# phaistos-networks/Trinity

Hardware: AMD Instinct MI355X
Metric: queries/sec (higher is better)
Workload: dtype u32

## Files before the change

### trinity_amd/csrc/k_score.hpp

```cpp
#pragma once
#include "k_match.hpp"

#ifndef TRI_SCORE_TILE
#define TRI_SCORE_TILE 4096
#endif
constexpr uint32_t SCORE_TILE = TRI_SCORE_TILE;
constexpr uint32_t TOPK_CAP = TOPK_MAX + AND_WG;

struct TopK {
        double s[TOPK_CAP];
        uint32_t d[TOPK_CAP];
        uint32_t n;
        uint32_t full;
        double thr_s;
        uint32_t thr_d;
};

__device__ __forceinline__ bool better(const double s1, const uint32_t d1, const double s2, const uint32_t d2) {
        return s1 > s2 || (s1 == s2 && d1 < d2);
}

__device__ void topk_prune(TopK &tk, const uint32_t k, uint32_t *scan) {
        const uint32_t tid = threadIdx.x;
        const uint32_t n = uni(tk.n);
// ... 337 lines not shown
                                                       float *__restrict__ top_scores, uint32_t *__restrict__ top_counts) {
        __shared__ TopK tk;
        __shared__ uint32_t scan[8];
        const uint32_t tid = threadIdx.x;
        for (uint32_t slot = blockIdx.x; slot < nq; slot += gridDim.x) {
                const DevQuery q = plan[slot];
                if (q.qid == 0xffffffffu)
                        continue;
                tk.n = 0;
                tk.full = 0;
                __syncthreads();
                for (uint32_t t = 0; t < q.ntasks; ++t) {
                        const uint32_t tix = q.first_task + t;
                        const uint32_t c = part_counts[tix];
                        for (uint32_t base = 0; base < c; base += AND_WG) {
                                const uint32_t i = base + tid;
                                const bool v = i < c;
                                topk_offer(tk, k, v, v ? part_scores[(uint64_t)tix * k + i] : 0.0, v ? part_docs[(uint64_t)tix * k + i] : 0u, scan);
                        }
                }
                topk_prune(tk, k, scan);
                const uint32_t n = uni(tk.n);
                for (uint32_t i = tid; i < k; i += AND_WG) {
                        top_docs[(uint64_t)q.qid * k + i] = i < n ? tk.d[i] : 0u;
                        top_scores[(uint64_t)q.qid * k + i] = i < n ? (float)tk.s[i] : 0.0f;
                }
                if (uni(tid >> 6) == 0)
                        top_counts[q.qid] = n;
                __syncthreads();
        }
}

__global__ void k_query_counts(const DevQuery *__restrict__ plan, const uint32_t *__restrict__ counts_by_task, const uint32_t nq,
                               uint64_t *__restrict__ qcounts) {
        const uint32_t s = blockIdx.x * blockDim.x + threadIdx.x;
        if (s >= nq)
                return;
        const DevQuery q = plan[s];
        if (q.qid == 0xffffffffu)
                return;
        uint64_t c = 0;
        for (uint32_t t = 0; t < q.ntasks; ++t)
                c += counts_by_task[q.first_task + t];
        qcounts[q.qid] = c;
}

struct DevSource {
        const DevQuery *plan;
        const uint32_t *slot_of_query;
        const uint32_t *part_docs;
        const double *part_scores;
        const uint32_t *part_counts;
        const uint64_t *qcounts;
};
__global__ __launch_bounds__(AND_WG) void k_topk_merge_sources(const DevSource *__restrict__ src, const uint32_t nsrc, const uint32_t nq, const uint32_t k,
                                                               uint32_t *__restrict__ top_docs, float *__restrict__ top_scores,
                                                               uint32_t *__restrict__ top_counts, uint64_t *__restrict__ counts) {
        __shared__ TopK tk;
        __shared__ uint32_t scan[8];
        const uint32_t tid = threadIdx.x;
        for (uint32_t qi = blockIdx.x; qi < nq; qi += gridDim.x) {
                tk.n = 0;
                tk.full = 0;
                __syncthreads();
                uint64_t total = 0;
                for (uint32_t s = 0; s < nsrc; ++s) {
                        const DevSource S = src[s];
// ... 134 lines not shown
```

### trinity_amd/csrc/trinity_hip.hip

```cpp
#include "../../include/trinity_hip.h"
#include <chrono>
#include <hip/hip_runtime.h>

#include <algorithm>
#include <array>
#include <cmath>
#include <cstdarg>
#include <cstdio>
#include <cstring>
#include <ctime>
#include <unistd.h>
#include <dlfcn.h>
#include <memory>
#include <mutex>
#include <numeric>
#include <string>
#include <thread>
#include <unordered_map>
#include <functional>
#include <vector>

static thread_local char g_err[512] = "";
static int fail(int code, const char *fmt, ...) {
        va_list ap;
// ... 256 lines not shown
struct tri_filter {
        DevRef dev;
        tri_index *ix = nullptr;
        Pooled<uint32_t> d_bits;
        size_t words = 0;
        ~tri_filter() {
                if (dev)
                        hipSetDevice(dev->device);
        }
};
struct tri_column {
        DevRef dev;
        tri_index *ix = nullptr;
        DevMem<uint32_t> d_values;
        uint32_t n = 0;
        ~tri_column() {
                if (dev)
                        hipSetDevice(dev->device);
        }
};
static size_t filter_words(const tri_index *ix) { return ((size_t)ix->max_doc / SPAN_BITS + 2) * SPAN_WORDS; }

enum BatchEvent { EV_UP, EV_START, EV_PLANE_ROWS, EV_DENSE, EV_PSET, EV_PROBE, EV_CAND, EV_FUSED, EV_PLANES, EV_PHRASE, EV_TREE, EV_END, EV_COUNT };

struct tri_batch : BatchPlan {
        DevRef dev;
        tri_index *ix = nullptr;
        uint32_t flags, topk;
        int similarity = TRI_SIM_BM25;
        size_t nq;
        Pinned<uint8_t> pinned;
        Pooled<uint8_t> d_arena;
        PooledEvent ev[EV_COUNT];
        Pooled<uint32_t> d_sparse;
        Pooled<uint32_t> d_out;
        Pooled<uint32_t> d_rich_allow;
        DevMem<uint64_t> d_hashes;
        Pooled<uint32_t> d_part_docs;
        Pooled<double> d_part_scores, d_all_scores;
        Pooled<uint32_t> d_rich_present;
        Pooled<uint16_t> d_rich_freq;
        Pooled<uint16_t> d_rich_freq_wide;
        Pooled<uint32_t> d_rich_present_hi, d_rich_allow_hi;
        DevMem<uint16_t> d_rich_pool;
        DevMem<uint8_t> d_rich_plen;
        DevMem<uint64_t> d_rich_payload;
        Pooled<double> d_pscore;
        Pooled<uint32_t> d_tree_scratch;
        Pooled<double> d_tree_scores;
        Pooled<uint32_t> d_scat_docs;
        Pooled<uint8_t> d_filter_tab;
        Pooled<uint32_t> d_filter_rows;
        Pooled<uint8_t> d_rank_block;
        Pooled<uint32_t> d_facet_rows;
        PooledEvent facet_ev[2];
        Pooled<uint64_t> d_order_block;
        DevMem<DevOrderGroup> d_order_groups;
        PooledEvent order_ev[2];
        template <class T>
        T *dev_at(const Span<T> &s) const {
                return reinterpret_cast<T *>(d_arena + s.off);
        }
        template <class T>
        T *dev_opt(const Span<T> &s) const {
                return s.empty() ? nullptr : dev_at(s);
        }
// ... 704 lines not shown
                        plan_lock = std::unique_lock<std::mutex>(dev->planners[0].mu);
                }
                tri_dev::PlanCtx &pc = dev->planners[which];
                if (nq >= 1024 && !pc.pool) {
                        const unsigned budget = host_cpu_budget();
                        const unsigned fair = budget >= 10 ? std::min(16u, (budget - 4) / tri_dev::PLAN_CTXS) : budget >= 4 ? 2u : 1u;
                        const unsigned want = dev->opt.plan_threads ? (unsigned)std::min<uint64_t>(dev->opt.plan_threads, 64) : fair;
                        if (want > 1) {
                                try {
                                        DevLock g(dev->mu);
                                        pc.pool = std::make_unique<HostPool>(want, dev->opt.plan_pin != 0, (unsigned)dev->opt.plan_hot_us, which, tri_dev::PLAN_CTXS, dev->plan_anchor, dev->opt.plan_pin == 2);
                                        if (dev->plan_anchor < 0)
                                                dev->plan_anchor = pc.pool->anchor();
                                } catch (...) {
                                }
                        }
                }
                rc = plan_batch(*ix, env, in, pc.pool.get(), [&](size_t bytes) { return b->pinned.alloc(dev, bytes); }, *b, err, &pc.frag_cache);
        } catch (const std::bad_alloc &) {
                return fail(TRI_ERR_NOMEM, "tri_batch_create: out of host memory");
        }
        if (rc != TRI_OK)
                return fail(rc, "%s", err.c_str());
        if (!b->last_unsupported.empty())
                fail(TRI_ERR_UNSUPPORTED, "%s", b->last_unsupported.c_str());
        return TRI_OK;
}

static size_t batch_arena(tri_batch *b, uint8_t *base, size_t *zero_from) {
        const size_t nt = b->tasks.size(), np = b->plan.size(), nq = b->nq, topk = b->topk;
        const bool scored = batch_scored(b), rich = batch_rich(b), scatter = b->pscatter_queries;
        Carver carve{base, b->block_bytes};
        carve(b->d_counts, (nt + 1) * 4);
        carve(b->d_ticket, TICKET_BYTES);
        carve(b->d_build, (b->plane_terms.size() + 1) * 8);
        carve(b->d_qthr, (np + 1) * 8, b->n_planes + b->n_planes8 != 0);
        carve(b->d_part_counts, (nt + 1) * 4, scored);
        carve(b->d_score_order, (nt + 1) * 4, scored);
        carve(b->d_task_hits, (nt + 1) * 4, rich);
        carve(b->d_task_pos_base, (nt + 1) * 8, rich);
        carve(b->d_scat_off, (nt + 1) * 4, scatter);
        carve(b->d_scat_cnt, (nt + 1) * 4, scatter);
        carve(b->d_scat_list, (b->pscatter_queries + 1) * 4, scatter);
        *zero_from = carve.at;
        carve(b->d_qcounts, (nq + 1) * 8);
        carve(b->d_top_counts, (nq + 1) * 4, scored);
        carve(b->d_top_docs, (nq * topk + 1) * 4, scored);
        carve(b->d_top_scores, (nq * topk + 1) * 4, scored);
        return carve.at;
}

static int create_arena(tri_batch *b) {
        tri_dev *dev = b->dev;
        size_t a_zero = 0;
        const size_t a = batch_arena(b, nullptr, &a_zero);
        HIP_TRY(b->d_arena.alloc(dev, a + 256));
        batch_arena(b, b->d_arena, &a_zero);
        if (b->pscatter_queries) {
                if (b->pscatter_docs + 64 > 0xffffffffull)
                        return fail(TRI_ERR_UNSUPPORTED, "tri_batch_create: the unions' terms without a plane hold more than 2^32 documents");
                b->scat_cap = (uint32_t)b->pscatter_docs;
                HIP_TRY(b->d_scat_docs.alloc(dev, ((size_t)b->scat_cap + 64) * 4));
        }
        for (PooledEvent &e : b->ev)
                HIP_TRY(e.take(dev));
        if (b->block_bytes)
                HIP_TRY(hipMemcpyAsync(b->d_arena, b->block, b->block_bytes, hipMemcpyHostToDevice, dev->stream_up));
        HIP_TRY(hipMemsetAsync(b->d_arena + a_zero, 0, a - a_zero, dev->stream_up));
        return TRI_OK;
}

static size_t tree_scratch(tri_batch *b, uint32_t *base) {
        const size_t plw = b->plw, nterms = b->tree_terms.size(), nhid = b->tree_hidden.size(), nchunks = (plw + TREE_CHUNK_WORDS - 1) / TREE_CHUNK_WORDS;
        Carver carve{reinterpret_cast<uint8_t *>(base), 0, 4};
        carve(b->d_tree_rows, nterms * PL_PLANES * plw * 4);
        carve(b->d_tree_prows, nhid * plw * 4);
        carve(b->d_tree_qbits, (size_t)b->n_tree * plw * 4);
// ... 95 lines not shown
        };
        auto b = std::make_unique<tri_batch>();
        b->ix = ix;
        b->dev.retain(dev);
        b->flags = flags;
        b->topk = topk;
        b->similarity = similarity;
        b->nq = nq;
        const PlanInput in{prog, prog_len, queries, nq, weights, flags, topk, similarity};
        if (const int rc = create_plan(b.get(), in))
                return rc;
        dbg_lap(0);
        DevLock dev_lock(dev->mu);
        if (const int rc = create_arena(b.get()))
                return rc;
        dbg_lap(1);
        if (const int rc = create_buffers(b.get(), in, dbg_lap))
                return rc;
        HIP_TRY(hipEventRecord(b->ev[EV_UP], dev->stream_up));
        create_info(b.get());
        b->info.create_ms = (float)std::chrono::duration<double, std::milli>(std::chrono::steady_clock::now() - t_create).count();
        if (dbg_create)
                fprintf(stderr, "[tri create] nq %zu: plan %.3f  arena+copy %.3f  planes/sparse %.3f  out(%.1f MB) %.3f  rest %.3f  total %.3f ms\n", nq, dbg_t[0], dbg_t[1] - dbg_t[0],
                        dbg_t[2] - dbg_t[1], (double)b->out_capacity * 4 / 1e6, dbg_t[3] - dbg_t[2], b->info.create_ms - dbg_t[3], b->info.create_ms);
        *out = b.release();
        return TRI_OK;
}

extern "C" void tri_batch_destroy(tri_batch *b) {
        delete b;
}


static FilterSel filter_sel(const tri_batch *b) {
        if (b->filter_rows.empty())
                return FilterSel{nullptr, nullptr, nullptr, 0u};
        return FilterSel{b->d_filter_rows, (const uint32_t *)b->d_filter_tab.get(), b->dev_at(b->tasks), (uint32_t)filter_words(b->ix)};
}
template <class F>
struct FilteredKernel;
template <class... A>
struct FilteredKernel<void (*)(A...)> {
        using type = void (*)(A..., FilterSel);
};
template <class Pick, class... Args>
static void tri_launch_matching(const tri_batch *b, const int kernel, const int variant, Pick pick, const dim3 grid, const dim3 block, const hipStream_t stream, Args &&...args) {
        const FilterSel fsel = filter_sel(b);
        if (!fsel.rows)
                return tri_launch(b->ix->codec, pick, grid, block, stream, std::forward<Args>(args)...);
        using Plain = decltype(+pick(std::integral_constant<int, CODEC_GOOGLE>()));
        const auto twin = reinterpret_cast<typename FilteredKernel<Plain>::type>(const_cast<void *>(filtered_kernel(kernel, b->ix->codec == TRI_CODEC_LUCENE ? CODEC_LUCENE : CODEC_GOOGLE, variant)));
        hipLaunchKernelGGL(twin, grid, block, 0, stream, std::forward<Args>(args)..., fsel);
}
static size_t filter_tab_ptrs_off(const tri_batch *b) { return (b->plan.size() * 4 + 15) & ~(size_t)15; }

static int run_filter_rows(tri_batch *b) {
        if (b->filter_rows.empty())
                return TRI_OK;
        tri_dev *dev = b->dev;
        const size_t n4 = filter_words(b->ix) / 4;
        const uint32_t nrows = (uint32_t)b->filter_rows.size();
        for (uint32_t y0 = 0; y0 < nrows; y0 += 65535u) {
                hipLaunchKernelGGL(k_filter_rows, dim3((unsigned)std::min<size_t>((n4 + FILTER_WG - 1) / FILTER_WG, 1024), std::min(65535u, nrows - y0)), dim3(FILTER_WG), 0, dev->stream,
                                   (const uint4 *const *)(b->d_filter_tab + filter_tab_ptrs_off(b)) + y0, (const uint4 *)b->ix->d_masked.get(), (uint4 *)b->d_filter_rows.get() + (size_t)y0 * n4, n4);
                HIP_TRY(hipGetLastError());
        }
        return TRI_OK;
}

static int run_plane_rows(tri_batch *b) {
        tri_dev *dev = b->dev;
        tri_index *ix = b->ix;
        b->info.term_planes_decoded_bytes = 0;
        if (!b->plane_terms.empty()) {
                std::vector<uint32_t> build;
                const uint8_t needs = b->planes_hi ? 3u : 1u;
                for (const uint32_t term : b->plane_terms) {
                        const uint32_t row = ix->df_rank[term];
                        if (row < ix->pc_cap && ((ix->pc_built[row] & needs) != needs || dev->opt.planes_rebuild)) {
                                build.push_back(term);
                                build.push_back(row);
                                b->info.term_planes_decoded_bytes += ix->docbytes[term];
                        }
                }
                if (!build.empty()) {
                        HIP_TRY(hipMemcpyAsync(b->d_build, build.data(), build.size() * 4, hipMemcpyHostToDevice, dev->stream));
                        const uint32_t nrows = (uint32_t)(build.size() / 2), nwin = b->plw / PL_WORDS;
                        for (uint32_t y0 = 0; y0 < nrows; y0 += 65535u) {
                                const uint32_t ny = std::min(65535u, nrows - y0);
                                if (b->planes_hi)
                                        TRI_LAUNCH(k_term_planes, ix->codec, dim3(nwin, ny), dim3(AND_WG), dev->stream, ix->d_index, ix->d_blk_last, ix->d_blk_off, ix->d_blk_rec,
                                                   ix->d_blk_doff, ix->d_win, ix->d_terms, (const uint32_t *)b->d_build + 2 * (size_t)y0, ix->d_pcache, (size_t)b->plw, ix->d_pcache_hi,
                                                   (size_t)PL_HI * b->plw, b->plw, (uint32_t *)nullptr);
                                else
                                        TRI_LAUNCH(k_term_plane0, ix->codec, dim3((nwin + P0_GROUP - 1) / P0_GROUP, ny), dim3(AND_WG), dev->stream, ix->d_index, ix->d_blk_last, ix->d_blk_off,
                                                   ix->d_blk_rec, ix->d_blk_doff, ix->d_win, ix->d_terms, (const uint32_t *)b->d_build + 2 * (size_t)y0, ix->d_pcache, b->plw, (uint32_t *)nullptr);
                                HIP_TRY(hipGetLastError());
                        }
                        for (size_t i = 1; i < build.size(); i += 2)
                                ix->pc_built[build[i]] |= needs;
                }
        }
        HIP_TRY(hipEventRecord(b->ev[EV_PLANE_ROWS], dev->stream));
        return TRI_OK;
}

static int run_matching(tri_batch *b) {
        tri_dev *dev = b->dev;
        tri_index *ix = b->ix;
        const uint8_t *match_bytes = ix->codec == TRI_CODEC_GOOGLE ? ix->d_dstream : ix->d_index;
        const uint32_t *match_off = ix->codec == TRI_CODEC_GOOGLE ? ix->d_blk_doff : ix->d_blk_off;
        uint32_t dense_wgs = TRI_DENSE_WAVES * 256 / DENSE_WG, cand_wgs = 4;
        bool overlap = false;
        if (dev->opt.overlap_dense_wgs && dev->opt.overlap_cand_wgs && (b->n_dense || b->n_pset) && b->n_cand) {
                overlap = true;
                dense_wgs = (uint32_t)dev->opt.overlap_dense_wgs;
                cand_wgs = (uint32_t)dev->opt.overlap_cand_wgs;
        } else if (dev->opt.overlap && b->n_cand && trip::sched_first(*b, TASK_CAND))
                overlap = true;
        hipStream_t cand_stream = dev->stream;
        if (overlap) {
                HIP_TRY(hipEventRecord(dev->ev_fork, dev->stream));
                HIP_TRY(hipStreamWaitEvent(dev->stream2, dev->ev_fork, 0));
                cand_stream = dev->stream2;
        }
        const DevPsetUnit *units = b->dev_at(b->units);
        const uint32_t *pset_sched = b->dev_at(b->pset_sched);
        const FilterSel fsel = filter_sel(b);
        const bool prep = b->n_pset && b->pscatter_queries, prep_forked = prep && !overlap && b->n_dense;
        if (prep) {
                if (prep_forked) {
                        HIP_TRY(hipEventRecord(dev->ev_fork, dev->stream));
                        HIP_TRY(hipStreamWaitEvent(dev->stream2, dev->ev_fork, 0));
                }
                hipStream_t prep_stream = prep_forked ? dev->stream2 : dev->stream;
                const uint32_t nunits = b->n_pset + b->n_probe, nscat = (uint32_t)b->pscatter_queries;
                hipLaunchKernelGGL(k_psets_prep_list, dim3((nunits + 255) / 256), dim3(256), 0, prep_stream, units, nunits, b->d_ticket + TICKET_SCAT_WORD + 1, b->d_scat_list, nscat);
                HIP_TRY(hipGetLastError());
                TRI_LAUNCH(k_psets_prep, ix->codec, dim3(nscat), dim3(PSCAT_WG), prep_stream, units, (const uint32_t *)b->d_scat_list, (const uint32_t *)(b->d_ticket + TICKET_SCAT_WORD + 1),
                           b->dev_at(b->plan), b->dev_at(b->tasks), (const uint32_t *)b->dev_at(b->qterms), (const uint32_t *)b->dev_opt(b->qplane), ix->d_masked, ix->d_index, ix->d_blk_last, ix->d_blk_off, ix->d_blk_rec,
                           ix->d_blk_doff, ix->d_terms, b->d_ticket + TICKET_SCAT_WORD, b->d_scat_off, b->d_scat_cnt, b->d_scat_docs, b->scat_cap, fsel);
                HIP_TRY(hipGetLastError());
                if (prep_forked)
                        HIP_TRY(hipEventRecord(dev->ev_join, dev->stream2));
        }
        if (b->n_dense) {
                tri_launch_matching(b, FK_AND_DENSE, 0, [](auto c) { return k_and_dense<c.value>; }, dim3(std::min<uint32_t>(b->n_dense, (uint32_t)dev->cus * dense_wgs)), dim3(DENSE_WG), dev->stream, match_bytes, ix->d_blk_last,
                           match_off, ix->d_win, ix->d_terms, b->dev_at(b->plan), b->dev_at(b->tasks), b->dev_at(b->sched) + trip::sched_first(*b, TASK_DENSE), b->dev_at(b->qterms), b->n_dense,
                           b->d_ticket + TICKET_DENSE_WORD, b->d_out, b->d_counts, ix->d_masked, (const uint32_t *)b->dev_opt(b->qplane), (const uint32_t *)ix->d_pcache, b->plw);
                HIP_TRY(hipGetLastError());
        }
        HIP_TRY(hipEventRecord(b->ev[EV_DENSE], dev->stream));
        if (prep_forked)
                HIP_TRY(hipStreamWaitEvent(dev->stream, dev->ev_join, 0));
        if (b->n_pset) {
                const uint32_t pset_wgs = TRI_PSET_WAVES * 256 / PSET_WG;
                tri_launch_matching(b, FK_PSETS, 0, [](auto c) { return k_psets<c.value>; }, dim3(std::min<uint32_t>(b->n_pset, (uint32_t)dev->cus * (overlap && dev->opt.overlap_dense_wgs ? std::min<uint32_t>(dense_wgs, pset_wgs) : pset_wgs))),
                           dim3(PSET_WG), dev->stream, units, pset_sched, b->n_pset, b->d_ticket + TICKET_PSET_WORD, (const uint32_t *)b->dev_at(b->qterms), (const uint32_t *)b->dev_opt(b->qplane), b->d_out,
                           b->d_counts, ix->d_masked, (const uint32_t *)ix->d_pcache, b->plw, (const uint32_t *)b->d_scat_off, (const uint32_t *)b->d_scat_cnt,
                           (const uint32_t *)b->d_scat_docs);
                HIP_TRY(hipGetLastError());
        }
        HIP_TRY(hipEventRecord(b->ev[EV_PSET], dev->stream));
        if (b->n_probe) {
                tri_launch_matching(b, FK_PROBE, 0, [](auto c) { return k_probe<c.value>; }, dim3(std::min<uint32_t>((b->n_probe + PROBE_WG / 64 - 1) / (PROBE_WG / 64), (uint32_t)dev->cus * (TRI_PROBE_WAVES * 256 / PROBE_WG))),
                           dim3(PROBE_WG), dev->stream, match_bytes, ix->d_blk_last, match_off, ix->d_terms, units, pset_sched + b->n_pset, b->n_probe, b->d_ticket + TICKET_PROBE_WORD,
                           (const uint32_t *)b->dev_at(b->qterms), (const uint32_t *)b->dev_opt(b->qplane), b->d_out, b->d_counts, ix->d_masked, (const uint32_t *)ix->d_pcache, b->plw);
                HIP_TRY(hipGetLastError());
        }
        HIP_TRY(hipEventRecord(b->ev[EV_PROBE], dev->stream));
        if (b->n_cand)
                tri_launch_matching(b, FK_AND, 0, [](auto c) { return k_and<c.value>; }, dim3(std::min<uint32_t>(b->n_cand, (uint32_t)dev->cus * cand_wgs)), dim3(AND_WG), cand_stream, match_bytes, ix->d_blk_last, match_off,
                           ix->d_win, ix->d_terms, b->dev_at(b->plan), b->dev_at(b->tasks), b->dev_at(b->sched) + trip::sched_first(*b, TASK_CAND), b->dev_at(b->qterms), b->dev_at(b->cand_q),
                           b->d_ticket + TICKET_CAND_WORD, b->d_out, b->d_counts, ix->d_masked, (const uint32_t *)b->dev_opt(b->qplane), (const uint32_t *)ix->d_pcache, b->plw);
        HIP_TRY(hipGetLastError());
        if (overlap) {
                HIP_TRY(hipEventRecord(dev->ev_join, dev->stream2));
                HIP_TRY(hipStreamWaitEvent(dev->stream, dev->ev_join, 0));
        }
        HIP_TRY(hipEventRecord(b->ev[EV_CAND], dev->stream));
        return TRI_OK;
}

static int run_fused(tri_batch *b) {
        tri_dev *dev = b->dev;
        tri_index *ix = b->ix;
        for (uint32_t kind = TASK_FUSED; kind <= TASK_FUSED_GEN; ++kind) {
                const uint32_t nf = b->*trip::SCHED_COUNT[kind], variant = kind - TASK_FUSED;
                if (!nf)
                        continue;
                tri_launch_matching(b, FK_FUSED, (int)variant, [&](auto c) { return std::array{k_fused<c.value, 0, 0>, k_fused<c.value, 1, 0>, k_fused<c.value, 0, 1>}[variant]; },
                           dim3(std::min<uint32_t>(nf, (uint32_t)dev->cus * FUS_WGS_PER_CU)), dim3(FUS_WG), dev->stream, ix->d_index, ix->d_blk_last, ix->d_blk_off, ix->d_blk_rec,
                           ix->d_blk_doff, ix->d_win, ix->d_terms, b->dev_at(b->plan), b->dev_at(b->fused), b->dev_at(b->tasks), (const uint32_t *)b->dev_at(b->sched) + trip::sched_first(*b, kind), b->dev_at(b->sterms),
                           b->dev_at(b->sweights), nf, b->d_ticket + TICKET_FUSED_WORD + 2 * variant, b->d_counts, b->topk, b->d_part_docs, b->d_part_scores, b->d_part_counts, ix->d_masked,
                           b->similarity, b->d_out, b->d_all_scores, b->d_rich_allow);
                HIP_TRY(hipGetLastError());
        }
        HIP_TRY(hipEventRecord(b->ev[EV_FUSED], dev->stream));
        return TRI_OK;
}

static int run_planes(tri_batch *b) {
        tri_dev *dev = b->dev;
        tri_index *ix = b->ix;
        if (b->d_qthr)
                HIP_TRY(hipMemsetAsync(b->d_qthr, 0, (b->plan.size() + 1) * 8, dev->stream));
        for (uint32_t kind = TASK_PLANES; kind <= TASK_PLANES8; ++kind) {
                const uint32_t np = b->*trip::SCHED_COUNT[kind], wide = kind - TASK_PLANES;
                if (!np)
                        continue;
                tri_launch_matching(b, FK_PLANES, (int)wide, [&](auto c) { return wide ? k_planes<c.value, FUS_MAX_SLOTS> : k_planes<c.value, PLK_NS_SMALL>; },
                           dim3(std::min<uint32_t>(np, (uint32_t)dev->cus * PLK_WGS_PER_CU)), dim3(PLK_WG), dev->stream, ix->d_index, ix->d_blk_last, ix->d_blk_off, ix->d_blk_rec,
                           ix->d_blk_doff, ix->d_win, ix->d_terms, b->dev_at(b->plan), b->dev_at(b->fused), b->dev_at(b->tasks), (const uint32_t *)b->dev_at(b->sched) + trip::sched_first(*b, kind), b->dev_at(b->sterms),
                           b->dev_at(b->sweights), np, b->d_ticket + TICKET_PLANES_WORD + 2 * wide, b->d_counts, b->topk, b->d_part_docs, b->d_part_scores, b->d_part_counts, ix->d_masked,
                           b->similarity, (const uint32_t *)ix->d_pcache, (const uint32_t *)ix->d_pcache_hi, b->plw, ix->pc_cap, b->d_sparse, b->sparse_cap, b->d_qthr);
                HIP_TRY(hipGetLastError());
        }
        HIP_TRY(hipEventRecord(b->ev[EV_PLANES], dev->stream));
        return TRI_OK;
}

static int run_phrases(tri_batch *b) {
        tri_dev *dev = b->dev;
        tri_index *ix = b->ix;
        if (!b->ptasks.empty() && ix->codec == TRI_CODEC_GOOGLE && ix->d_prank && ix->pc_cap) {
                std::vector<uint32_t> hits_build, hits_only;
                uint32_t max_blocks = 0;
                for (size_t i = 0; i < b->pterms.size(); ++i) {
                        const uint32_t term = b->pterms[i], r = ix->df_rank[term];
                        if (r >= ix->pc_cap || ix->ph_built[r])
                                continue;
                        const DevTerm &t = ix->terms[term];
                        if (!(t.flags & TERM_FULL_BLOCKS) || !t.documents)
                                continue;
                        ix->ph_built[r] = 1;
                        max_blocks = std::max(max_blocks, t.nblocks);
                        std::vector<uint32_t> &dst = (ix->pc_built[r] & 4u) ? hits_only : hits_build;
                        ix->pc_built[r] |= 5u;
                        dst.push_back(term);
                        dst.push_back(r);
                }
                const uint32_t nrows_build = (uint32_t)(hits_build.size() / 2);
                hits_build.insert(hits_build.end(), hits_only.begin(), hits_only.end());
                if (!hits_build.empty()) {
                        uint32_t *d_pairs = ix->d_ph_pairs + 2 * ix->ph_pairs_n;
                        HIP_TRY(hipMemcpyAsync(d_pairs, hits_build.data(), hits_build.size() * 4, hipMemcpyHostToDevice, dev->stream));
                        ix->ph_pairs_n += hits_build.size() / 2;
                        for (uint32_t y0 = 0; y0 < nrows_build; y0 += 65535u) {
                                const dim3 grid((b->plw / PL_WORDS + P0_GROUP - 1) / P0_GROUP, std::min(65535u, nrows_build - y0));
                                TRI_LAUNCH(k_term_plane0, ix->codec, grid, dim3(AND_WG), dev->stream, ix->d_index, ix->d_blk_last, ix->d_blk_off, ix->d_blk_rec, ix->d_blk_doff, ix->d_win,
                                           ix->d_terms, (const uint32_t *)d_pairs + 2 * (size_t)y0, ix->d_pcache, b->plw, ix->d_prank);
                                HIP_TRY(hipGetLastError());
                        }
                        const uint32_t npairs = (uint32_t)(hits_build.size() / 2);
                        for (uint32_t y0 = 0; y0 < npairs; y0 += 65535u) {
                                hipLaunchKernelGGL(k_term_hits, dim3((max_blocks + 255) / 256, std::min(65535u, npairs - y0)), dim3(256), 0, dev->stream, ix->d_index, ix->d_blk_off,
                                                   ix->d_blk_hits, ix->d_terms, (const uint32_t *)d_pairs + 2 * (size_t)y0, (const uint64_t *)ix->d_hs_off, ix->d_phs, ix->d_term_row);
                                HIP_TRY(hipGetLastError());
                        }
                }
        }
        if (!b->ptasks.empty()) {
                const uint32_t np = (uint32_t)b->ptasks.size();
                TRI_LAUNCH(k_phrase, ix->codec, dim3(std::min<uint32_t>(np, (uint32_t)dev->cus * PHRASE_WGS_PER_CU)), dim3(AND_WG), dev->stream, ix->d_index, ix->d_hits,
                           ix->d_blk_hits, ix->d_hdir, ix->d_blk_last, ix->d_blk_off, ix->d_win, ix->d_terms, b->dev_at(b->plan), b->dev_at(b->tasks), b->dev_at(b->ptasks), np, b->dev_at(b->phrases), b->dev_at(b->pterms),
                           b->d_ticket + TICKET_PHRASE_WORD, b->d_out, b->d_counts, b->d_pscore,
                           (b->flags & TRI_FLAG_ACCUMULATED_SCORE) ? 65535u : 1u,
                           b->similarity, (const uint32_t *)ix->d_pcache, ix->pc_plw, (const uint32_t *)ix->d_prank, (const unsigned long long *)ix->d_phs,
                           (const uint64_t *)ix->d_hs_off, ix->codec == TRI_CODEC_GOOGLE ? (const uint32_t *)ix->d_term_row : nullptr);
                HIP_TRY(hipGetLastError());
        }
        HIP_TRY(hipEventRecord(b->ev[EV_PHRASE], dev->stream));
        return TRI_OK;
}

static int run_trees(tri_batch *b) {
        tri_dev *dev = b->dev;
        tri_index *ix = b->ix;
        if (b->n_tree) {
                const uint32_t plw = b->plw, nterms = (uint32_t)b->tree_terms.size(), nhid = (uint32_t)b->tree_hidden.size();
                const uint32_t nchunks = (plw + TREE_CHUNK_WORDS - 1) / TREE_CHUNK_WORDS;
                const uint32_t *tsched = b->dev_at(b->sched) + trip::sched_first(*b, TASK_TREE);
                const uint32_t *d_tree = b->dev_at(b->tree);
                for (uint32_t y0 = 0; y0 < nterms; y0 += 65535u) {
                        const dim3 grid(plw / PL_WORDS, std::min(65535u, nterms - y0));
                        TRI_LAUNCH(k_term_planes, ix->codec, grid, dim3(AND_WG), dev->stream, ix->d_index, ix->d_blk_last, ix->d_blk_off, ix->d_blk_rec, ix->d_blk_doff, ix->d_win,
                                   ix->d_terms, (const uint32_t *)b->d_tree_build + 2 * (size_t)y0, b->d_tree_rows, (size_t)PL_PLANES * plw, b->d_tree_rows + plw,
                                   (size_t)PL_PLANES * plw, plw, (uint32_t *)nullptr);
                        HIP_TRY(hipGetLastError());
                }
                if (nhid) {
                        HIP_TRY(hipMemsetAsync(b->d_tree_prows, 0, (size_t)nhid * plw * 4, dev->stream));
                        hipLaunchKernelGGL(k_tree_gather, dim3(nhid), dim3(TREE_WG), 0, dev->stream, b->dev_at(b->plan), b->dev_at(b->tasks), b->dev_at(b->tree_hidden), b->d_out,
                                           b->d_counts, b->d_pscore, b->d_tree_prows, plw);
                        HIP_TRY(hipGetLastError());
                }
                const bool scored_run = b->flags & TRI_FLAG_ACCUMULATED_SCORE, rich_run = b->flags & TRI_FLAG_MATCHED_TERMS;
                double *tscores = !scored_run ? nullptr : b->topk ? (double *)b->d_tree_scores : (double *)b->d_all_scores;
                const uint32_t n_narrow = b->n_tree - b->n_tree_wide;
                for (uint32_t y0 = 0; y0 < b->n_tree;) {
                        const bool wide = y0 >= n_narrow;
                        const uint32_t ny = std::min(65535u, (wide ? b->n_tree : n_narrow) - y0);
                        const dim3 grid(nchunks, ny);
                        uint32_t *qbits = b->d_tree_qbits + (size_t)y0 * plw, *cc = b->d_tree_cc + (size_t)y0 * nchunks;
#define TREE_EVAL_ARGS b->dev_at(b->plan), b->dev_at(b->tasks), tsched + y0, d_tree, (const uint32_t *)b->d_tree_rows, (const uint32_t *)b->d_tree_prows, (const uint32_t *)ix->d_masked, qbits, cc, plw, filter_sel(b)
                        if (wide)
                                hipLaunchKernelGGL(k_tree_eval_wide, grid, dim3(TREE_WG), 0, dev->stream, TREE_EVAL_ARGS);
                        else
                                hipLaunchKernelGGL(k_tree_eval, grid, dim3(TREE_WG), 0, dev->stream, TREE_EVAL_ARGS);
#undef TREE_EVAL_ARGS
                        hipLaunchKernelGGL(k_tree_expand, grid, dim3(TREE_WG), 0, dev->stream, b->dev_at(b->plan), b->dev_at(b->tasks), tsched + y0, (const uint32_t *)qbits, (const uint32_t *)cc,
                                           b->d_out, b->d_counts, plw);
                        if (scored_run || rich_run) {
#define TREE_LEAVES_ARGS                                                                                                                                                                   \
        ix->d_index, ix->d_blk_last, ix->d_blk_off, ix->d_terms, b->dev_at(b->plan), b->dev_at(b->tasks), tsched + y0, d_tree, (const uint32_t *)b->d_tree_rows,                          \
                (const uint32_t *)b->d_tree_prows, (const uint32_t *)cc, (const uint32_t *)b->d_out, (const uint32_t *)b->d_counts, (const double *)b->dev_at(b->sweights),               \
                (const double *)b->d_pscore, tscores, rich_run ? (uint32_t *)b->d_rich_allow : nullptr, plw, b->similarity, b->d_rich_allow_hi,                                                     \
                (const DevRichWide *)b->dev_opt(b->rich_wide)
                                if (wide)
                                        TRI_LAUNCH(k_tree_leaves_wide, ix->codec, grid, dim3(TREE_WG), dev->stream, TREE_LEAVES_ARGS);
                                else
                                        TRI_LAUNCH(k_tree_leaves, ix->codec, grid, dim3(TREE_WG), dev->stream, TREE_LEAVES_ARGS);
#undef TREE_LEAVES_ARGS
                        }
                        HIP_TRY(hipGetLastError());
                        y0 += ny;
                }
                if (scored_run && b->topk) {
                        hipLaunchKernelGGL(k_tree_topk, dim3(b->n_tree), dim3(AND_WG), 0, dev->stream, tsched, b->dev_at(b->tasks), (const uint32_t *)b->d_out, (const uint32_t *)b->d_counts,
                                           (const double *)tscores, b->topk, b->d_part_docs, b->d_part_scores, b->d_part_counts);
                        HIP_TRY(hipGetLastError());
                }
        }
        HIP_TRY(hipEventRecord(b->ev[EV_TREE], dev->stream));
        return TRI_OK;
}

template <bool WRITE>
static int launch_rich(tri_batch *b) {
        tri_dev *dev = b->dev;
        tri_index *ix = b->ix;
        const uint32_t n_wide = b->n_rich_wide, n = (uint32_t)b->tasks.size() - n_wide;
        const uint32_t *sched = n_wide ? b->dev_at(b->rich_sched) : b->dev_at(b->sched);
        const RichWideArgs wd{b->d_rich_present_hi, b->d_rich_allow_hi, b->d_rich_freq_wide, b->dev_opt(b->rich_wide)};
#define RICH_ARGS(SCHED, N, TICKET)                                                                                                                                                        \
        ix->d_index, ix->d_hits, ix->d_blk_hits, ix->d_hdir, ix->d_pdir, ix->d_blk_last, ix->d_blk_off, ix->d_terms, b->dev_at(b->plan), b->dev_at(b->tasks), SCHED, b->dev_at(b->sterms), N,         \
                b->d_ticket + (WRITE ? TICKET_RICH_WRITE_WORD : TICKET_RICH_COUNT_WORD) + TICKET, b->d_out, b->d_counts, b->rich_R, b->d_rich_present, b->d_rich_freq, b->d_task_hits,     \
                WRITE ? (const uint64_t *)b->d_task_pos_base : nullptr, WRITE ? (uint16_t *)b->d_rich_pool : nullptr, (const uint32_t *)b->d_rich_allow, WRITE ? (uint8_t *)b->d_rich_plen : nullptr,             \
                WRITE ? (uint64_t *)b->d_rich_payload : nullptr
        if (n)
                tri_launch(ix->codec, [](auto c) { return k_rich<c.value, WRITE>; }, dim3(std::min<uint32_t>(n, (uint32_t)dev->cus * 3)), dim3(AND_WG), dev->stream, RICH_ARGS(sched, n, 0));
        if (n_wide)
                tri_launch(ix->codec, [](auto c) { return k_rich_wide<c.value, WRITE>; }, dim3(std::min<uint32_t>(n_wide, (uint32_t)dev->cus * 3)), dim3(AND_WG), dev->stream,
                           RICH_ARGS(sched + n, n_wide, TICKET_RICH_WIDE), wd);
#undef RICH_ARGS
        HIP_TRY(hipGetLastError());
        return TRI_OK;
}

static int run_rich_count(tri_batch *b) {
        if (!(b->flags & TRI_FLAG_MATCHED_TERMS))
                return TRI_OK;
        tri_dev *dev = b->dev;
        HIP_TRY(hipMemsetAsync(b->d_rich_present, 0, (b->out_capacity + 64) * 4, dev->stream));
        HIP_TRY(hipMemsetAsync(b->d_rich_freq, 0, (b->out_capacity + 64) * 2 * b->rich_R, dev->stream));
        HIP_TRY(hipMemsetAsync(b->d_task_hits, 0, (b->tasks.size() + 1) * 4, dev->stream));
        if (b->n_rich_wide) {
                HIP_TRY(hipMemsetAsync(b->d_rich_present_hi, 0, (b->rich_wide_slots + 64) * 4, dev->stream));
                HIP_TRY(hipMemsetAsync(b->d_rich_freq_wide, 0, (b->rich_wide_cells + 64) * 2, dev->stream));
        }
        return launch_rich<false>(b);
}

static int run_scores(tri_batch *b) {
        if (!(b->flags & TRI_FLAG_ACCUMULATED_SCORE))
                return TRI_OK;
        tri_dev *dev = b->dev;
        tri_index *ix = b->ix;
        const uint32_t nlegacy = trip::sched_first(*b, TASK_FUSED);
        if (nlegacy) {
                hipLaunchKernelGGL(k_score_order, dim3(1), dim3(SORD_WG), 0, dev->stream, (const uint32_t *)b->dev_at(b->sched), (const uint32_t *)b->d_counts, nlegacy, b->d_score_order);
                HIP_TRY(hipGetLastError());
                TRI_LAUNCH(k_score, ix->codec, dim3(std::min<uint32_t>(nlegacy, (uint32_t)dev->cus * SCORE_WGS_PER_CU)), dim3(AND_WG), dev->stream, ix->d_index, ix->d_blk_last,
                           ix->d_blk_off, ix->d_terms, b->dev_at(b->plan), b->dev_at(b->tasks), (const uint32_t *)b->d_score_order, b->dev_at(b->sterms), b->dev_at(b->sweights), nlegacy,
                           b->d_ticket + TICKET_SCORE_WORD, b->d_out, b->d_counts, b->topk, b->d_part_docs, b->d_part_scores, b->d_part_counts, b->d_all_scores, b->d_pscore,
                           b->similarity, ix->d_win, b->dev_opt(b->splane),
                           (const uint32_t *)ix->d_pcache_hi, b->plw);
        }
        HIP_TRY(hipGetLastError());
        const uint32_t nqs = (uint32_t)b->plan.size();
        if (b->topk)
                hipLaunchKernelGGL(k_topk_merge, dim3(std::min<uint32_t>(nqs, (uint32_t)dev->cus * 8)), dim3(AND_WG), 0, dev->stream, b->dev_at(b->plan), nqs, b->topk, b->d_part_docs,
                                   b->d_part_scores, b->d_part_counts, b->d_top_docs, b->d_top_scores, b->d_top_counts);
        HIP_TRY(hipGetLastError());
        return TRI_OK;
}

static int run_query_counts(tri_batch *b) {
        if (!b->plan.empty()) {
                const uint32_t nqs = (uint32_t)b->plan.size();
                hipLaunchKernelGGL(k_query_counts, dim3((nqs + 255) / 256), dim3(256), 0, b->dev->stream, b->dev_at(b->plan), b->d_counts, nqs, b->d_qcounts);
                HIP_TRY(hipGetLastError());
        }
        return TRI_OK;
}

static int run_facets(tri_batch *b) {
        b->facet_ran = b->facet_done = false;
        if (!b->facets.n)
                return TRI_OK;
        tri_dev *dev = b->dev;
        HIP_TRY(hipEventRecord(b->facet_ev[0], dev->stream));
        HIP_TRY(hipMemsetAsync(b->d_facet_rows, 0, b->facet_counters * 4, dev->stream));
        if (!b->tasks.empty()) {
                hipLaunchKernelGGL(k_facet, dim3((uint32_t)b->tasks.size()), dim3(FACET_WG), 0, dev->stream, (const DevQuery *)b->dev_at(b->plan), (const DevTask *)b->dev_at(b->tasks),
                                   (const uint32_t *)b->d_counts, (const uint32_t *)b->d_out, b->facets, b->d_facet_rows.get());
                HIP_TRY(hipGetLastError());
        }
        HIP_TRY(hipEventRecord(b->facet_ev[1], dev->stream));
        b->facet_ran = true;
        return TRI_OK;
}

static int run_order(tri_batch *b) {
        b->order_ran = b->order_done = false;
        if (!b->order_on)
                return TRI_OK;
        tri_dev *dev = b->dev;
        const uint32_t k = b->order.topk;
        const size_t ntasks = b->tasks.size(), rows = b->order_lists;
        HIP_TRY(hipEventRecord(b->order_ev[0], dev->stream));
        if (b->tasks.empty()) {
                HIP_TRY(hipMemsetAsync(b->order_keys(rows), 0, b->nq * (size_t)k * 8, dev->stream));
                HIP_TRY(hipMemsetAsync(b->order_counts(rows), 0, b->nq * 4, dev->stream));
// ... 22 lines not shown
        tri_dev *dev = b->dev;
        DevLock dev_lock(dev->mu);
        HIP_TRY(hipSetDevice(dev->device));
        b->synced = false;
        b->rank_done = false;
#ifdef TRI_TRACE
        if (!g_trace_host) {
                HIP_TRY(hipHostMalloc((void **)&g_trace_host, 64 * 16, hipHostMallocMapped | hipHostMallocCoherent));
                uint32_t *dptr = nullptr;
                HIP_TRY(hipHostGetDevicePointer((void **)&dptr, g_trace_host, 0));
                HIP_TRY(hipMemcpyToSymbol(HIP_SYMBOL(g_trace), &dptr, sizeof dptr));
        }
        memset(g_trace_host, 0, 64 * 16);
#endif
        b->ran = true;
#ifdef TRI_TASKTIMES
        if (b->tasks.size()) {
                if (g_tt_cap < 8 * (size_t)b->tasks.size()) {
                        if (g_tt_host)
                                hipHostFree(g_tt_host);
                        g_tt_cap = 8 * (size_t)b->tasks.size() + 1024;
                        HIP_TRY(hipHostMalloc((void **)&g_tt_host, g_tt_cap * 8, hipHostMallocMapped | hipHostMallocCoherent));
                        unsigned long long *dptr = nullptr;
                        HIP_TRY(hipHostGetDevicePointer((void **)&dptr, g_tt_host, 0));
                        HIP_TRY(hipMemcpyToSymbol(HIP_SYMBOL(g_tt), &dptr, sizeof dptr));
                }
                memset(g_tt_host, 0, g_tt_cap * 8);
        }
#endif
        HIP_TRY(hipStreamWaitEvent(dev->stream, b->ev[EV_UP], 0));
        if (b->ix->ev_pc_ready)
                HIP_TRY(hipStreamWaitEvent(dev->stream, b->ix->ev_pc_ready, 0));
        HIP_TRY(hipEventRecord(b->ev[EV_START], dev->stream));
        if (b->tasks.empty()) {
                for (int e = EV_PLANE_ROWS; e <= EV_TREE; ++e)
                        HIP_TRY(hipEventRecord(b->ev[e], dev->stream));
        } else {
                HIP_TRY(hipMemsetAsync(b->d_ticket, 0, TICKET_BYTES, dev->stream));
                for (int (*stage)(tri_batch *) : {run_filter_rows, run_plane_rows, run_matching, run_fused, run_planes, run_phrases, run_trees, run_rich_count, run_scores})
                        if (const int rc = stage(b))
                                return rc;
        }
        if (const int rc = run_query_counts(b))
                return rc;
        if (const int rc = run_facets(b))
                return rc;
        if (const int rc = run_order(b))
                return rc;
        HIP_TRY(hipEventRecord(b->ev[EV_END], dev->stream));
        return TRI_OK;
}

#ifdef TRI_TASKTIMES
static void report_tasktimes(tri_batch *b) {
        const tri_dev *dev = b->dev;
        if (!b->tasks.size() || !getenv("TRINITY_TASKTIMES"))
                return;
#if TRI_TASKTIMES == 2
        const uint32_t nc = trip::sched_first(*b, TASK_FUSED), first = 0;
#elif TRI_TASKTIMES == 5
        const uint32_t nc = (uint32_t)b->ptasks.size(), first = 0;
#elif TRI_TASKTIMES == 4
        const uint32_t nc = b->n_dense, first = trip::sched_first(*b, TASK_DENSE);
#elif TRI_TASKTIMES == 3
        const uint32_t nc = b->n_planes, first = trip::sched_first(*b, TASK_PLANES);
#else
        const uint32_t nc = b->n_cand, first = trip::sched_first(*b, TASK_CAND);
#endif
        unsigned long long t0 = ~0ull, t1 = 0, busy = 0;
        std::vector<std::pair<unsigned long long, uint32_t>> by;
        for (uint32_t i = 0; i < nc; ++i) {
                const unsigned long long s = g_tt_host[8 * i], e = g_tt_host[8 * i + 1];
                if (!s || !e)
                        continue;
                t0 = std::min(t0, s), t1 = std::max(t1, e);
                busy += e - s;
                by.emplace_back(e - s, i);
        }
        std::sort(by.rbegin(), by.rend());
        const double span_us = (double)(t1 - t0) / 100.0;
        const unsigned wgs = std::min<uint32_t>(nc, (uint32_t)dev->cus * (TRI_TASKTIMES == 3 ? PLK_WGS_PER_CU : TRI_TASKTIMES == 2 ? SCORE_WGS_PER_CU : TRI_TASKTIMES == 5 ? PHRASE_WGS_PER_CU : 4));
        fprintf(stderr, "[tri tasktimes] k_and: %u tasks, span %.1f us, busy %.1f %% of %u workgroups; mean task %.2f us\n", nc, span_us,
// ... 93 lines not shown
                const DevTask &tk = b->tasks[ti];
                const DevQuery &q = b->plan[tk.slot];
                std::string tt;
                char buf[96];
                if (task_onepass(tk.kind)) {
                        const DevFused &z = b->fused[q.fused_idx];
                        for (uint32_t j = 0; j < z.nslots; ++j) {
                                snprintf(buf, sizeof buf, " %u(df %u%s)", z.term[j], b->ix->terms[z.term[j]].documents, z.plane[j] != PL_NONE ? " plane" : "");
                                tt += buf;
                        }
                        snprintf(buf, sizeof buf, " nreq %u", z.nreq);
                        tt += buf;
                } else
                for (uint32_t j = 0; j < q.nterms; ++j) {
                        const uint32_t term = b->qterms[q.term_base + j] & QT_TERM;
                        snprintf(buf, sizeof buf, " %s%u(df %u%s)", (b->qterms[q.term_base + j] & QT_GROUP) ? "|" : "", term, b->ix->terms[term].documents,
                                 (!b->qplane.empty() && b->qplane[q.term_base + j] != PL_NONE) ? " plane" : "");
                        tt += buf;
                }
                snprintf(buf, sizeof buf, "  matches %u phrases %u", b->h_counts.empty() ? 0u : b->h_counts[ti], q.nphrases);
                tt += buf;
                fprintf(stderr, "   %.1f us (started %.1f us in)  ticket %u  tiles [%u, %u)  query %u:%s\n", (double)by[k].first / 100.0,
                        (double)(g_tt_host[8 * by[k].second] - t0) / 100.0, by[k].second, tk.tile_begin, tk.tile_end, q.qid, tt.c_str());
                fprintf(stderr, "        last tile: lead decoded +%.1f us", ((double)g_tt_host[8 * by[k].second + 2] - (double)g_tt_host[8 * by[k].second]) / 100.0);
                for (int j = 3; j < 8; ++j)
                        if (g_tt_host[8 * by[k].second + j])
                                fprintf(stderr, "  term %d +%.1f", j - 2, ((double)g_tt_host[8 * by[k].second + j] - (double)g_tt_host[8 * by[k].second]) / 100.0);
                fprintf(stderr, "\n");
        }
}
#endif

static void read_stage_times(tri_batch *b) {
        static const struct { BatchEvent from; float tri_batch_info::*ms; } STAGES[] = {
                {EV_START, &tri_batch_info::term_planes_ms}, {EV_PLANE_ROWS, &tri_batch_info::dense_ms}, {EV_DENSE, &tri_batch_info::pset_ms}, {EV_PSET, &tri_batch_info::probe_ms},
                {EV_PROBE, &tri_batch_info::cand_ms}, {EV_CAND, &tri_batch_info::fused_ms}, {EV_FUSED, &tri_batch_info::planes_ms}, {EV_PLANES, &tri_batch_info::phrase_ms},
                {EV_PHRASE, &tri_batch_info::tree_ms}, {EV_TREE, &tri_batch_info::rest_ms}};
        float ms = 0;
        if (hipEventElapsedTime(&ms, b->ev[EV_START], b->ev[EV_END]) == hipSuccess)
                b->info.last_run_ms = ms;
        for (const auto &s : STAGES) {
                b->info.*s.ms = 0;
                if (!b->tasks.empty() && hipEventElapsedTime(&ms, b->ev[s.from], b->ev[s.from + 1]) == hipSuccess)
                        b->info.*s.ms = ms;
        }
}

static int account_matches(tri_batch *b) {
        b->h_counts.resize(b->tasks.size());
        if (!b->tasks.empty())
                HIP_TRY(hipMemcpy(b->h_counts.data(), b->d_counts, b->tasks.size() * 4, hipMemcpyDeviceToHost));
        const bool sc = b->flags & TRI_FLAG_ACCUMULATED_SCORE;
        uint64_t m = 0, m_kind[TASK_KINDS] = {}, out_kind[TASK_KINDS] = {};
        b->h_query_counts.assign(b->plan.size(), 0);
        for (size_t sidx = 0; sidx < b->plan.size(); ++sidx) {
                const DevQuery &q = b->plan[sidx];
                for (uint32_t t = 0; t < q.ntasks; ++t)
                        b->h_query_counts[sidx] += b->h_counts[q.first_task + t];
                if (q.qid == 0xffffffffu)
                        continue;
                const uint64_t c = b->h_query_counts[sidx];
                m += c;
                if (!q.ntasks)
                        continue;
                const uint32_t kind = b->tasks[q.first_task].kind;
                m_kind[kind] += c;
                if (task_onepass(kind))
                        out_kind[kind] += q.out_cap ? 4 * c : 8 * std::min<uint64_t>(c, b->topk);
                else if (kind != TASK_TREE)
                        out_kind[kind] += sc && b->topk ? 8 * std::min<uint64_t>(c, b->topk) : (kind == TASK_DENSE || kind == TASK_PSET) && q.form == RESULT_BITMAP ? 4ull * q.out_cap : 4 * c;
        }
        const uint64_t out_fused = out_kind[TASK_FUSED] + out_kind[TASK_FUSED16] + out_kind[TASK_FUSED_GEN], out_planes = out_kind[TASK_PLANES] + out_kind[TASK_PLANES8];
        b->info.dense_algorithmic_bytes = b->term_bytes_dense + 4 * m_kind[TASK_DENSE];
        b->info.pset_algorithmic_bytes = b->term_bytes_pset + 4 * m_kind[TASK_PSET];
        b->info.pset_queries = b->pset_queries;
        b->info.probe_algorithmic_bytes = b->term_bytes_probe + 4 * m_kind[TASK_PROBE];
        b->info.probe_queries = b->probe_queries;
        b->info.cand_algorithmic_bytes = (b->term_bytes - b->term_bytes_dense - b->term_bytes_pset - b->term_bytes_probe - b->term_bytes_fused - b->term_bytes_planes - b->term_bytes_phrase_hits) + 4 * m_kind[TASK_CAND];
// ... 856 lines not shown
```

Before: 14.54 million.

## Skip event records for empty stages and clear tickets in query-count kernel

Stage events are now recorded only when a stage actually enqueued work, which removes the many hipEventRecord calls per run, and stage timings are rebuilt from whichever events were recorded. The per-run ticket memset is replaced by having block 0 of k_query_counts zero the ticket words at the end of each run, so later runs skip the memset. The ticket buffer moves out of the zeroed arena region. The cross-run ticket state is fragile: if a run fails partway, the armed flag stays false and the next run falls back to the memset.

New measurement: 15.04 million (median of 6 runs). 1.03x the previous value.

```diff
diff --git a/trinity_amd/csrc/k_score.hpp b/trinity_amd/csrc/k_score.hpp
--- a/trinity_amd/csrc/k_score.hpp
+++ b/trinity_amd/csrc/k_score.hpp
@@ -393,7 +393,10 @@
 }
 
 __global__ void k_query_counts(const DevQuery *__restrict__ plan, const uint32_t *__restrict__ counts_by_task, const uint32_t nq,
-                               uint64_t *__restrict__ qcounts) {
+                               uint64_t *__restrict__ qcounts, uint32_t *__restrict__ tickets, const uint32_t ticket_words) {
+        if (blockIdx.x == 0)
+                for (uint32_t w = threadIdx.x; w < ticket_words; w += blockDim.x)
+                        tickets[w] = 0u;
         const uint32_t s = blockIdx.x * blockDim.x + threadIdx.x;
         if (s >= nq)
                 return;
diff --git a/trinity_amd/csrc/trinity_hip.hip b/trinity_amd/csrc/trinity_hip.hip
--- a/trinity_amd/csrc/trinity_hip.hip
+++ b/trinity_amd/csrc/trinity_hip.hip
@@ -312,6 +312,9 @@
         Pinned<uint8_t> pinned;
         Pooled<uint8_t> d_arena;
         PooledEvent ev[EV_COUNT];
+        uint32_t ev_recorded = 0;
+        bool tickets_armed = true;
+        bool run_cleared_tickets = false;
         Pooled<uint32_t> d_sparse;
         Pooled<uint32_t> d_out;
         Pooled<uint32_t> d_rich_allow;
@@ -1082,7 +1085,6 @@
         const bool scored = batch_scored(b), rich = batch_rich(b), scatter = b->pscatter_queries;
         Carver carve{base, b->block_bytes};
         carve(b->d_counts, (nt + 1) * 4);
-        carve(b->d_ticket, TICKET_BYTES);
         carve(b->d_build, (b->plane_terms.size() + 1) * 8);
         carve(b->d_qthr, (np + 1) * 8, b->n_planes + b->n_planes8 != 0);
         carve(b->d_part_counts, (nt + 1) * 4, scored);
@@ -1093,6 +1095,7 @@
         carve(b->d_scat_cnt, (nt + 1) * 4, scatter);
         carve(b->d_scat_list, (b->pscatter_queries + 1) * 4, scatter);
         *zero_from = carve.at;
+        carve(b->d_ticket, TICKET_BYTES);
         carve(b->d_qcounts, (nq + 1) * 8);
         carve(b->d_top_counts, (nq + 1) * 4, scored);
         carve(b->d_top_docs, (nq * topk + 1) * 4, scored);
@@ -1254,6 +1257,14 @@
 }
 
 
+static int close_stage(tri_batch *b, const BatchEvent e, const bool enqueued) {
+        if (!enqueued)
+                return TRI_OK;
+        HIP_TRY(hipEventRecord(b->ev[e], b->dev->stream));
+        b->ev_recorded |= 1u << e;
+        return TRI_OK;
+}
+
 static FilterSel filter_sel(const tri_batch *b) {
         if (b->filter_rows.empty())
                 return FilterSel{nullptr, nullptr, nullptr, 0u};
@@ -1294,6 +1305,7 @@
         tri_dev *dev = b->dev;
         tri_index *ix = b->ix;
         b->info.term_planes_decoded_bytes = 0;
+        bool built = false;
         if (!b->plane_terms.empty()) {
                 std::vector<uint32_t> build;
                 const uint8_t needs = b->planes_hi ? 3u : 1u;
@@ -1306,6 +1318,7 @@
                         }
                 }
                 if (!build.empty()) {
+                        built = true;
                         HIP_TRY(hipMemcpyAsync(b->d_build, build.data(), build.size() * 4, hipMemcpyHostToDevice, dev->stream));
                         const uint32_t nrows = (uint32_t)(build.size() / 2), nwin = b->plw / PL_WORDS;
                         for (uint32_t y0 = 0; y0 < nrows; y0 += 65535u) {
@@ -1323,8 +1336,7 @@
                                 ix->pc_built[build[i]] |= needs;
                 }
         }
-        HIP_TRY(hipEventRecord(b->ev[EV_PLANE_ROWS], dev->stream));
-        return TRI_OK;
+        return close_stage(b, EV_PLANE_ROWS, built || !b->filter_rows.empty() || b->run_cleared_tickets);
 }
 
 static int run_matching(tri_batch *b) {
@@ -1372,7 +1384,8 @@
                            b->d_ticket + TICKET_DENSE_WORD, b->d_out, b->d_counts, ix->d_masked, (const uint32_t *)b->dev_opt(b->qplane), (const uint32_t *)ix->d_pcache, b->plw);
                 HIP_TRY(hipGetLastError());
         }
-        HIP_TRY(hipEventRecord(b->ev[EV_DENSE], dev->stream));
+        if (const int rc = close_stage(b, EV_DENSE, b->n_dense || prep))
+                return rc;
         if (prep_forked)
                 HIP_TRY(hipStreamWaitEvent(dev->stream, dev->ev_join, 0));
         if (b->n_pset) {
@@ -1383,14 +1396,16 @@
                            (const uint32_t *)b->d_scat_docs);
                 HIP_TRY(hipGetLastError());
         }
-        HIP_TRY(hipEventRecord(b->ev[EV_PSET], dev->stream));
+        if (const int rc = close_stage(b, EV_PSET, b->n_pset))
+                return rc;
         if (b->n_probe) {
                 tri_launch_matching(b, FK_PROBE, 0, [](auto c) { return k_probe<c.value>; }, dim3(std::min<uint32_t>((b->n_probe + PROBE_WG / 64 - 1) / (PROBE_WG / 64), (uint32_t)dev->cus * (TRI_PROBE_WAVES * 256 / PROBE_WG))),
                            dim3(PROBE_WG), dev->stream, match_bytes, ix->d_blk_last, match_off, ix->d_terms, units, pset_sched + b->n_pset, b->n_probe, b->d_ticket + TICKET_PROBE_WORD,
                            (const uint32_t *)b->dev_at(b->qterms), (const uint32_t *)b->dev_opt(b->qplane), b->d_out, b->d_counts, ix->d_masked, (const uint32_t *)ix->d_pcache, b->plw);
                 HIP_TRY(hipGetLastError());
         }
-        HIP_TRY(hipEventRecord(b->ev[EV_PROBE], dev->stream));
+        if (const int rc = close_stage(b, EV_PROBE, b->n_probe))
+                return rc;
         if (b->n_cand)
                 tri_launch_matching(b, FK_AND, 0, [](auto c) { return k_and<c.value>; }, dim3(std::min<uint32_t>(b->n_cand, (uint32_t)dev->cus * cand_wgs)), dim3(AND_WG), cand_stream, match_bytes, ix->d_blk_last, match_off,
                            ix->d_win, ix->d_terms, b->dev_at(b->plan), b->dev_at(b->tasks), b->dev_at(b->sched) + trip::sched_first(*b, TASK_CAND), b->dev_at(b->qterms), b->dev_at(b->cand_q),
@@ -1400,17 +1415,18 @@
                 HIP_TRY(hipEventRecord(dev->ev_join, dev->stream2));
                 HIP_TRY(hipStreamWaitEvent(dev->stream, dev->ev_join, 0));
         }
-        HIP_TRY(hipEventRecord(b->ev[EV_CAND], dev->stream));
-        return TRI_OK;
+        return close_stage(b, EV_CAND, b->n_cand);
 }
 
 static int run_fused(tri_batch *b) {
         tri_dev *dev = b->dev;
         tri_index *ix = b->ix;
+        bool launched = false;
         for (uint32_t kind = TASK_FUSED; kind <= TASK_FUSED_GEN; ++kind) {
                 const uint32_t nf = b->*trip::SCHED_COUNT[kind], variant = kind - TASK_FUSED;
                 if (!nf)
                         continue;
+                launched = true;
                 tri_launch_matching(b, FK_FUSED, (int)variant, [&](auto c) { return std::array{k_fused<c.value, 0, 0>, k_fused<c.value, 1, 0>, k_fused<c.value, 0, 1>}[variant]; },
                            dim3(std::min<uint32_t>(nf, (uint32_t)dev->cus * FUS_WGS_PER_CU)), dim3(FUS_WG), dev->stream, ix->d_index, ix->d_blk_last, ix->d_blk_off, ix->d_blk_rec,
                            ix->d_blk_doff, ix->d_win, ix->d_terms, b->dev_at(b->plan), b->dev_at(b->fused), b->dev_at(b->tasks), (const uint32_t *)b->dev_at(b->sched) + trip::sched_first(*b, kind), b->dev_at(b->sterms),
@@ -1418,19 +1434,22 @@
                            b->similarity, b->d_out, b->d_all_scores, b->d_rich_allow);
                 HIP_TRY(hipGetLastError());
         }
-        HIP_TRY(hipEventRecord(b->ev[EV_FUSED], dev->stream));
-        return TRI_OK;
+        return close_stage(b, EV_FUSED, launched);
 }
 
 static int run_planes(tri_batch *b) {
         tri_dev *dev = b->dev;
         tri_index *ix = b->ix;
-        if (b->d_qthr)
+        bool launched = false;
+        if (b->d_qthr) {
                 HIP_TRY(hipMemsetAsync(b->d_qthr, 0, (b->plan.size() + 1) * 8, dev->stream));
+                launched = true;
+        }
         for (uint32_t kind = TASK_PLANES; kind <= TASK_PLANES8; ++kind) {
                 const uint32_t np = b->*trip::SCHED_COUNT[kind], wide = kind - TASK_PLANES;
                 if (!np)
                         continue;
+                launched = true;
                 tri_launch_matching(b, FK_PLANES, (int)wide, [&](auto c) { return wide ? k_planes<c.value, FUS_MAX_SLOTS> : k_planes<c.value, PLK_NS_SMALL>; },
                            dim3(std::min<uint32_t>(np, (uint32_t)dev->cus * PLK_WGS_PER_CU)), dim3(PLK_WG), dev->stream, ix->d_index, ix->d_blk_last, ix->d_blk_off, ix->d_blk_rec,
                            ix->d_blk_doff, ix->d_win, ix->d_terms, b->dev_at(b->plan), b->dev_at(b->fused), b->dev_at(b->tasks), (const uint32_t *)b->dev_at(b->sched) + trip::sched_first(*b, kind), b->dev_at(b->sterms),
@@ -1438,8 +1457,7 @@
                            b->similarity, (const uint32_t *)ix->d_pcache, (const uint32_t *)ix->d_pcache_hi, b->plw, ix->pc_cap, b->d_sparse, b->sparse_cap, b->d_qthr);
                 HIP_TRY(hipGetLastError());
         }
-        HIP_TRY(hipEventRecord(b->ev[EV_PLANES], dev->stream));
-        return TRI_OK;
+        return close_stage(b, EV_PLANES, launched);
 }
 
 static int run_phrases(tri_batch *b) {
@@ -1492,8 +1510,7 @@
                            (const uint64_t *)ix->d_hs_off, ix->codec == TRI_CODEC_GOOGLE ? (const uint32_t *)ix->d_term_row : nullptr);
                 HIP_TRY(hipGetLastError());
         }
-        HIP_TRY(hipEventRecord(b->ev[EV_PHRASE], dev->stream));
-        return TRI_OK;
+        return close_stage(b, EV_PHRASE, !b->ptasks.empty());
 }
 
 static int run_trees(tri_batch *b) {
@@ -1554,8 +1571,7 @@
                         HIP_TRY(hipGetLastError());
                 }
         }
-        HIP_TRY(hipEventRecord(b->ev[EV_TREE], dev->stream));
-        return TRI_OK;
+        return close_stage(b, EV_TREE, b->n_tree);
 }
 
 template <bool WRITE>
@@ -1621,7 +1637,8 @@
 static int run_query_counts(tri_batch *b) {
         if (!b->plan.empty()) {
                 const uint32_t nqs = (uint32_t)b->plan.size();
-                hipLaunchKernelGGL(k_query_counts, dim3((nqs + 255) / 256), dim3(256), 0, b->dev->stream, b->dev_at(b->plan), b->d_counts, nqs, b->d_qcounts);
+                hipLaunchKernelGGL(k_query_counts, dim3((nqs + 255) / 256), dim3(256), 0, b->dev->stream, b->dev_at(b->plan), b->d_counts, nqs, b->d_qcounts, b->d_ticket,
+                                   (uint32_t)(TICKET_BYTES / 4));
                 HIP_TRY(hipGetLastError());
         }
         return TRI_OK;
@@ -1710,11 +1727,12 @@
         if (b->ix->ev_pc_ready)
                 HIP_TRY(hipStreamWaitEvent(dev->stream, b->ix->ev_pc_ready, 0));
         HIP_TRY(hipEventRecord(b->ev[EV_START], dev->stream));
-        if (b->tasks.empty()) {
-                for (int e = EV_PLANE_ROWS; e <= EV_TREE; ++e)
-                        HIP_TRY(hipEventRecord(b->ev[e], dev->stream));
-        } else {
-                HIP_TRY(hipMemsetAsync(b->d_ticket, 0, TICKET_BYTES, dev->stream));
+        b->ev_recorded = 0;
+        if (!b->tasks.empty()) {
+                b->run_cleared_tickets = !b->tickets_armed;
+                b->tickets_armed = false;
+                if (b->run_cleared_tickets)
+                        HIP_TRY(hipMemsetAsync(b->d_ticket, 0, TICKET_BYTES, dev->stream));
                 for (int (*stage)(tri_batch *) : {run_filter_rows, run_plane_rows, run_matching, run_fused, run_planes, run_phrases, run_trees, run_rich_count, run_scores})
                         if (const int rc = stage(b))
                                 return rc;
@@ -1726,6 +1744,8 @@
         if (const int rc = run_order(b))
                 return rc;
         HIP_TRY(hipEventRecord(b->ev[EV_END], dev->stream));
+        if (!b->tasks.empty())
+                b->tickets_armed = true;
         return TRI_OK;
 }
 
@@ -1885,18 +1905,25 @@
 #endif
 
 static void read_stage_times(tri_batch *b) {
-        static const struct { BatchEvent from; float tri_batch_info::*ms; } STAGES[] = {
-                {EV_START, &tri_batch_info::term_planes_ms}, {EV_PLANE_ROWS, &tri_batch_info::dense_ms}, {EV_DENSE, &tri_batch_info::pset_ms}, {EV_PSET, &tri_batch_info::probe_ms},
-                {EV_PROBE, &tri_batch_info::cand_ms}, {EV_CAND, &tri_batch_info::fused_ms}, {EV_FUSED, &tri_batch_info::planes_ms}, {EV_PLANES, &tri_batch_info::phrase_ms},
-                {EV_PHRASE, &tri_batch_info::tree_ms}, {EV_TREE, &tri_batch_info::rest_ms}};
+        static const struct { BatchEvent closes; float tri_batch_info::*ms; } STAGES[] = {
+                {EV_PLANE_ROWS, &tri_batch_info::term_planes_ms}, {EV_DENSE, &tri_batch_info::dense_ms}, {EV_PSET, &tri_batch_info::pset_ms}, {EV_PROBE, &tri_batch_info::probe_ms},
+                {EV_CAND, &tri_batch_info::cand_ms}, {EV_FUSED, &tri_batch_info::fused_ms}, {EV_PLANES, &tri_batch_info::planes_ms}, {EV_PHRASE, &tri_batch_info::phrase_ms},
+                {EV_TREE, &tri_batch_info::tree_ms}};
         float ms = 0;
         if (hipEventElapsedTime(&ms, b->ev[EV_START], b->ev[EV_END]) == hipSuccess)
                 b->info.last_run_ms = ms;
+        BatchEvent from = EV_START;
         for (const auto &s : STAGES) {
                 b->info.*s.ms = 0;
-                if (!b->tasks.empty() && hipEventElapsedTime(&ms, b->ev[s.from], b->ev[s.from + 1]) == hipSuccess)
+                if (!(b->ev_recorded >> s.closes & 1u))
+                        continue;
+                if (hipEventElapsedTime(&ms, b->ev[from], b->ev[s.closes]) == hipSuccess)
                         b->info.*s.ms = ms;
-        }
+                from = s.closes;
+        }
+        b->info.rest_ms = 0;
+        if (!b->tasks.empty() && hipEventElapsedTime(&ms, b->ev[from], b->ev[EV_END]) == hipSuccess)
+                b->info.rest_ms = ms;
 }
 
 static int account_matches(tri_batch *b) {
```
